# lucidrains/transfusion-pytorch

Measured on NVIDIA H100. Metric: train tokens/sec (text+latent) at d=512 L=8 seq=1024, higher is better.
Workload: dtype bf16

## Files before the change

### transfusion_pytorch_b200/csrc/gemm_sm90.cuh

```cuda
#pragma once
#include "sm90_ptx.cuh"
#include "dropout.cuh"

namespace tfx {

constexpr int GEMM_BM = 128;
constexpr int GEMM_BN = 128;
constexpr int GEMM_BK = 64;
constexpr int GEMM_UK = 16;

enum : int { EPI_STORE = 0, EPI_QKVG = 1, EPI_RESID = 2, EPI_GEGLU = 3, EPI_GEGLU_DROP = 4 };

struct GemmParams {
  int M, N, K;
  int k_splits;
  float* out_f32; long long ld_f32;
  __nv_bfloat16* out_bf16; long long ld_bf16;
  const float* bias;
  const long long* row_off;
  float alpha;
  int accumulate_f32;
  int K1;
  int H;
  __nv_bfloat16 *q, *k, *v;
  float* gates;
  float* mix_pre;
  float* qk_inv;
  const float *q_gamma, *k_gamma;
  const int* rope_pos;
  const float2* rope_cs;
  int rope_len;
  const int* kv_rows;
  const float* x_res; float* x_out; __nv_bfloat16* x_out_bf16;
  __nv_bfloat16* y_bf16;
  const int* cond_row;
  const float* zgate;
  long long zgate_ld;
  const float* ls;
  __nv_bfloat16* vg;
  __nv_bfloat16* h;
  DropParams drop;
};

template <int EPI> struct GemmCfg {
  static constexpr int THREADS = 384;
  static constexpr int STAGES = 4;
  static constexpr int A_BYTES = GEMM_BM * GEMM_BK * 2;
  static constexpr int B_BYTES = GEMM_BN * GEMM_BK * 2;
  static constexpr int STAGE_BYTES = A_BYTES + B_BYTES;
  static constexpr int ACC_BYTES = GEMM_BM * GEMM_BN * 4;
  static constexpr int STG_WARP = EPI == 2 ? 4096 + 2048 : 4096;
  static constexpr int STAGING = (EPI >= 3 ? 8 : 4) * STG_WARP;
  static constexpr int SMEM_BYTES = STAGES * STAGE_BYTES + ACC_BYTES + STAGING + 1024  + 256 ;
  static_assert(SMEM_BYTES <= 227 * 1024, "shared memory of one block");
};

__device__ __forceinline__ uint32_t acc_off(int r, int col) { return r * 512 + ((((col >> 2) ^ (r & 7))) << 4) + (col & 3) * 4; }
__device__ __forceinline__ void acc_ld32(const uint8_t* acc, int r, int col, uint32_t (&v)[32]) {
#pragma unroll
  for (int q = 0; q < 8; ++q) {
    const uint4 t = *reinterpret_cast<const uint4*>(acc + r * 512 + ((((col >> 2) + q) ^ (r & 7)) << 4));
    v[4 * q] = t.x; v[4 * q + 1] = t.y; v[4 * q + 2] = t.z; v[4 * q + 3] = t.w;
  }
}

__device__ __forceinline__ void gelu_parts(float g, float& cdf, float& pdf) {
  const float ax = fabsf(g) * 0.70710678118654752f;
  const float t = __fdividef(1.f, fmaf(0.3275911f, ax, 1.f));
  const float E = __expf(-ax * ax);
  float poly = fmaf(1.061405429f, t, -1.453152027f);
  poly = fmaf(poly, t, 1.421413741f);
  poly = fmaf(poly, t, -0.284496736f);
  poly = fmaf(poly, t, 0.254829592f);
  const float h = 0.5f * poly * t * E;
  cdf = g >= 0.f ? 1.f - h : h;
  pdf = 0.3989422804014327f * E;
}
__device__ __forceinline__ float gelu_erf(float x) { float c, d; gelu_parts(x, c, d); return x * c; }
__device__ __forceinline__ float2 geglu_pair(float2 g, float2 v) {
  return make_float2(gelu_erf(g.x) * v.x, gelu_erf(g.y) * v.y);
}

__device__ __forceinline__ void cp_async16_zfill(void* smem, const void* gmem, bool valid) {
  const int sz = valid ? 16 : 0;
  asm volatile("cp.async.cg.shared.global [%0], [%1], 16, %2;" ::"r"(smem_u32(smem)), "l"(gmem), "r"(sz) : "memory");
}

__device__ __forceinline__ uint32_t pack_bf16(float a, float b) {
  __nv_bfloat162 t = __floats2bfloat162_rn(a, b);
  return *reinterpret_cast<uint32_t*>(&t);
}
__device__ __forceinline__ float2 unpack2_bf16_(uint32_t w) {
  __nv_bfloat162 t = *reinterpret_cast<__nv_bfloat162*>(&w);
  return __bfloat1622float2(t);
}

template <int CH>
__device__ __forceinline__ void stg_put(uint8_t* sw, int lane, const uint32_t* w) {
#pragma unroll
  for (int c = 0; c < CH; ++c)
    *reinterpret_cast<uint4*>(sw + lane * 128 + ((c ^ (lane & 7)) << 4)) = make_uint4(w[4 * c], w[4 * c + 1], w[4 * c + 2], w[4 * c + 3]);
}
template <int CH>
__device__ __forceinline__ void stg_get(const uint8_t* sw, int lane, uint32_t* w) {
#pragma unroll
  for (int c = 0; c < CH; ++c) {
    const uint4 t = *reinterpret_cast<const uint4*>(sw + lane * 128 + ((c ^ (lane & 7)) << 4));
    w[4 * c] = t.x; w[4 * c + 1] = t.y; w[4 * c + 2] = t.z; w[4 * c + 3] = t.w;
  }
}
template <int CH>
__device__ __forceinline__ void stg_store(const uint8_t* sw, int lane, uint8_t* g, long long pitch, int rows_valid) {
  constexpr int RPI = 32 / CH;
#pragma unroll
  for (int it = 0; it < 32 / RPI; ++it) {
    const int row = it * RPI + lane / CH, ch = lane % CH;
    if (row < rows_valid)
      *reinterpret_cast<uint4*>(g + row * pitch + ch * 16) = *reinterpret_cast<const uint4*>(sw + row * 128 + ((ch ^ (row & 7)) << 4));
  }
}
__device__ __forceinline__ void stg_fetch(int lane, const uint8_t* g, long long pitch, int rows_valid, uint4 (&t)[8]) {
#pragma unroll
  for (int it = 0; it < 8; ++it) {
    const int row = it * 4 + lane / 8, ch = lane % 8;
    t[it] = row < rows_valid ? *reinterpret_cast<const uint4*>(g + row * pitch + ch * 16) : make_uint4(0, 0, 0, 0);
  }
}
__device__ __forceinline__ void stg_fill(uint8_t* sw, int lane, const uint4 (&t)[8]) {
#pragma unroll
  for (int it = 0; it < 8; ++it) {
    const int row = it * 4 + lane / 8, ch = lane % 8;
    *reinterpret_cast<uint4*>(sw + row * 128 + ((ch ^ (row & 7)) << 4)) = t[it];
  }
}

__device__ __forceinline__ void stg_put_pack(uint8_t* sw, int lane, const float* y) {
#pragma unroll
  for (int c = 0; c < 4; ++c)
    *reinterpret_cast<uint4*>(sw + lane * 128 + ((c ^ (lane & 7)) << 4)) =
        make_uint4(pack_bf16(y[8 * c], y[8 * c + 1]), pack_bf16(y[8 * c + 2], y[8 * c + 3]), pack_bf16(y[8 * c + 4], y[8 * c + 5]), pack_bf16(y[8 * c + 6], y[8 * c + 7]));
}
__device__ __forceinline__ void stg64_put(uint8_t* sw, int lane, const uint32_t* w) {
#pragma unroll
  for (int c = 0; c < 4; ++c)
    *reinterpret_cast<uint4*>(sw + lane * 64 + ((c ^ ((lane >> 1) & 3)) << 4)) = make_uint4(w[4 * c], w[4 * c + 1], w[4 * c + 2], w[4 * c + 3]);
}
__device__ __forceinline__ void stg64_put_pack(uint8_t* sw, int lane, const float* y) {
#pragma unroll
  for (int c = 0; c < 4; ++c)
    *reinterpret_cast<uint4*>(sw + lane * 64 + ((c ^ ((lane >> 1) & 3)) << 4)) =
        make_uint4(pack_bf16(y[8 * c], y[8 * c + 1]), pack_bf16(y[8 * c + 2], y[8 * c + 3]), pack_bf16(y[8 * c + 4], y[8 * c + 5]), pack_bf16(y[8 * c + 6], y[8 * c + 7]));
}
__device__ __forceinline__ void stg64_store(const uint8_t* sw, int lane, uint8_t* g, long long pitch, int rows_valid) {
#pragma unroll
  for (int it = 0; it < 4; ++it) {
    const int row = it * 8 + (lane >> 2), ch = lane & 3;
    if (row < rows_valid)
      *reinterpret_cast<uint4*>(g + row * pitch + ch * 16) = *reinterpret_cast<const uint4*>(sw + row * 64 + ((ch ^ ((row >> 1) & 3)) << 4));
  }
}

__device__ __forceinline__ void stg64_store_rows(const uint8_t* sw, int lane, uint8_t* g, long long pitch, int rows_valid, const int* __restrict__ rows) {
#pragma unroll
  for (int it = 0; it < 4; ++it) {
    const int row = it * 8 + (lane >> 2), ch = lane & 3;
    if (row < rows_valid)
      *reinterpret_cast<uint4*>(g + (long long)rows[row] * pitch + ch * 16) = *reinterpret_cast<const uint4*>(sw + row * 64 + ((ch ^ ((row >> 1) & 3)) << 4));
  }
}
template <int CH>
__device__ __forceinline__ void stg_store_rows(const uint8_t* sw, int lane, uint8_t* g, long long pitch, int rows_valid, const int* __restrict__ rows) {
  constexpr int RPI = 32 / CH;
#pragma unroll
  for (int it = 0; it < 32 / RPI; ++it) {
    const int row = it * RPI + lane / CH, ch = lane % CH;
    if (row < rows_valid)
      *reinterpret_cast<uint4*>(g + (long long)rows[row] * pitch + ch * 16) = *reinterpret_cast<const uint4*>(sw + row * 128 + ((ch ^ (row & 7)) << 4));
  }
}

template <class RowOf>
__device__ __forceinline__ void store_slice(const GemmParams& p, uint8_t* sw, int lane, uint32_t (&r)[32], int cbase, RowOf row_of) {
  const bool f32_staged = p.out_f32 && (p.row_off || (p.ld_f32 & 3) == 0) && ((reinterpret_cast<uintptr_t>(p.out_f32) & 15) == 0);
  const bool bf16_staged = p.out_bf16 && (p.ld_bf16 & 7) == 0 && ((reinterpret_cast<uintptr_t>(p.out_bf16) & 15) == 0);
  const int row = row_of(lane);
  const bool row_ok = row < p.M;
  const bool full = cbase + 32 <= p.N;
  float v[32];
#pragma unroll
  for (int j = 0; j < 32; ++j) v[j] = __uint_as_float(r[j]);
  if (p.alpha != 1.f) {
#pragma unroll
    for (int j = 0; j < 32; ++j) v[j] *= p.alpha;
  }
  if (p.bias) {
    if (full) {
#pragma unroll
      for (int j = 0; j < 32; j += 4) { const float4 b = *reinterpret_cast<const float4*>(p.bias + cbase + j); v[j] += b.x; v[j + 1] += b.y; v[j + 2] += b.z; v[j + 3] += b.w; }
    } else {
      for (int j = 0; j < 32; ++j) if (cbase + j < p.N) v[j] += p.bias[cbase + j];
    }
  }
  if (p.out_f32) {
    if (full && f32_staged) {
#pragma unroll
      for (int j = 0; j < 32; ++j) r[j] = __float_as_uint(v[j]);
      stg_put<8>(sw, lane, r);
      __syncwarp();
      auto put = [&](float* dst, float x) { if (p.accumulate_f32) atomicAdd(dst, x); else *dst = x; };
#pragma unroll
      for (int it = 0; it < 8; ++it) {
        const int rr = it * 4 + (lane >> 3), ch = lane & 7;
        const int grow = row_of(rr);
        if (grow < p.M) {
          const long long off = p.row_off ? p.row_off[grow] : (long long)grow * p.ld_f32;
          if (off >= 0) {
            float* drow = p.out_f32 + off + cbase;
            const uint8_t* srow = sw + rr * 128;
            const int a = (int)(reinterpret_cast<uintptr_t>(drow) >> 2) & 3;
            if (a == 0) {
              float* dst = drow + ch * 4;
              const float4 t = *reinterpret_cast<const float4*>(srow + ((ch ^ (rr & 7)) << 4));
              if (p.accumulate_f32) asm volatile("red.global.add.v4.f32 [%0], {%1, %2, %3, %4};" ::"l"(dst), "f"(t.x), "f"(t.y), "f"(t.z), "f"(t.w) : "memory");
              else *reinterpret_cast<float4*>(dst) = t;
            } else {
              const int pe = 4 - a;
              auto col = [&](int j) { return *reinterpret_cast<const float*>(srow + (((j >> 2) ^ (rr & 7)) << 4) + (j & 3) * 4); };
              if (ch < 7) {
                const int j = pe + 4 * ch;
                float* dst = drow + j;
                const float4 t = make_float4(col(j), col(j + 1), col(j + 2), col(j + 3));
                if (p.accumulate_f32) asm volatile("red.global.add.v4.f32 [%0], {%1, %2, %3, %4};" ::"l"(dst), "f"(t.x), "f"(t.y), "f"(t.z), "f"(t.w) : "memory");
                else *reinterpret_cast<float4*>(dst) = t;
              } else {
#pragma unroll
                for (int i = 0; i < 4; ++i) { const int j = i < pe ? i : 28 + i; put(drow + j, col(j)); }
              }
            }
          }
        }
      }
      __syncwarp();
    } else if (row_ok) {
      const long long off = p.row_off ? p.row_off[row] : (long long)row * p.ld_f32;
      if (off >= 0) {
        float* dst = p.out_f32 + off + cbase;
        for (int j = 0; j < 32; ++j)
          if (cbase + j < p.N) { if (p.accumulate_f32) atomicAdd(dst + j, v[j]); else dst[j] = v[j]; }
      }
    }
  }
  if (p.out_bf16) {
    if (full && bf16_staged) {
      uint32_t w[16];
#pragma unroll
      for (int j = 0; j < 16; ++j) w[j] = pack_bf16(v[2 * j], v[2 * j + 1]);
      stg_put<4>(sw, lane, w);
      __syncwarp();
#pragma unroll
      for (int it = 0; it < 4; ++it) {
        const int rr = it * 8 + (lane >> 2), ch = lane & 3;
        const int grow = row_of(rr);
        if (grow < p.M)
          *reinterpret_cast<uint4*>(p.out_bf16 + (long long)grow * p.ld_bf16 + cbase + ch * 8) = *reinterpret_cast<const uint4*>(sw + rr * 128 + ((ch ^ (rr & 7)) << 4));
      }
      __syncwarp();
    } else if (row_ok) {
      __nv_bfloat16* dst = p.out_bf16 + (long long)row * p.ld_bf16 + cbase;
      for (int j = 0; j < 32; ++j) if (cbase + j < p.N) dst[j] = __float2bfloat16(v[j]);
    }
  }
}

template <bool A_MN, bool B_MN, int EPI, int CL>
__global__ void __launch_bounds__(384, 1)
gemm_sm90_kernel(const __grid_constant__ CUtensorMap tmA, const __grid_constant__ CUtensorMap tmA2, const __grid_constant__ CUtensorMap tmB, const GemmParams p) {
  using Cfg = GemmCfg<EPI>;
  constexpr bool GEGLU = EPI == EPI_GEGLU || EPI == EPI_GEGLU_DROP;
  constexpr int BN = GEMM_BN;
  constexpr int STAGES = Cfg::STAGES;
  static_assert(Cfg::STAGE_BYTES % 1024 == 0 && 2 * STAGES <= 32, "stage alignment / barrier area");
  extern __shared__ __align__(1024) uint8_t smem_raw[];
  uint8_t* smem = smem_raw;
  if (threadIdx.x == 0 && (smem_u32(smem) & 1023u) != 0) __trap();
  uint8_t* acc = smem + STAGES * Cfg::STAGE_BYTES;
  uint8_t* staging = acc + Cfg::ACC_BYTES;
  uint64_t* bars = reinterpret_cast<uint64_t*>(staging + Cfg::STAGING);
  uint64_t* full_bar = bars;
  uint64_t* empty_bar = bars + STAGES;

  const int warp = threadIdx.x >> 5, lane = threadIdx.x & 31;
  const int m_tiles = (p.M + GEMM_BM - 1) / GEMM_BM;
  const int n_tiles = (p.N + BN - 1) / BN;
  const int kb_total = (p.K + GEMM_BK - 1) / GEMM_BK;
  const int kb_per_split = (kb_total + p.k_splits - 1) / p.k_splits;
  const int m_units = (m_tiles + CL - 1) / CL;
  const int unit_items = m_units * n_tiles;
  const int num_items = unit_items * p.k_splits;
  const int cta_rank = CL > 1 ? (int)cluster_ctarank() : 0;
  const int first_item = blockIdx.x / CL, item_stride = gridDim.x / CL;

  if (threadIdx.x == 0) {
    tma_prefetch_desc(&tmA);
    tma_prefetch_desc(&tmB);
    for (int s = 0; s < STAGES; ++s) { mbar_init(&full_bar[s], 1); mbar_init(&empty_bar[s], 4 * CL); }
    mbar_fence_init();
  }
  __syncthreads();
  if constexpr (CL > 1) cluster_sync_all();

  if (warp < 4) {
    setmaxnreg_dec<40>();
    if (threadIdx.x == 0) {
      int stage = 0; uint32_t phase = 0;
      for (int item = first_item; item < num_items; item += item_stride) {
        const int split = item / unit_items;
        const int rem = item - split * unit_items;
        const int m_unit = rem / n_tiles, n_blk = rem - m_unit * n_tiles;
        const int m_blk = m_unit * CL + cta_rank;
        const int kb0 = split * kb_per_split;
        const int kb1 = min(kb0 + kb_per_split, kb_total);
        for (int kb = kb0; kb < kb1; ++kb) {
          mbar_wait(&empty_bar[stage], phase ^ 1);
          uint8_t* sA = smem + stage * Cfg::STAGE_BYTES;
          uint8_t* sB = sA + Cfg::A_BYTES;
          mbar_expect_tx(&full_bar[stage], Cfg::STAGE_BYTES);
          if (!A_MN) {
            if (kb * GEMM_BK < p.K1) tma_load_2d(&tmA, &full_bar[stage], sA, kb * GEMM_BK, m_blk * GEMM_BM);
            else tma_load_2d(&tmA2, &full_bar[stage], sA, kb * GEMM_BK - p.K1, m_blk * GEMM_BM);
          } else {
#pragma unroll
            for (int a = 0; a < GEMM_BM / 64; ++a)
              tma_load_2d(&tmA, &full_bar[stage], sA + a * (GEMM_BK * 128), m_blk * GEMM_BM + a * 64, kb * GEMM_BK);
          }
          if constexpr (CL > 1) {
            if (!B_MN) tma_load_2d_multicast(&tmB, &full_bar[stage], sB + cta_rank * (64 * 128), kb * GEMM_BK, n_blk * BN + cta_rank * 64, (uint16_t)3);
            else tma_load_2d_multicast(&tmB, &full_bar[stage], sB + cta_rank * (GEMM_BK * 128), n_blk * BN + cta_rank * 64, kb * GEMM_BK, (uint16_t)3);
          } else if (!B_MN) {
            tma_load_2d(&tmB, &full_bar[stage], sB, kb * GEMM_BK, n_blk * BN);
          } else {
#pragma unroll
            for (int a = 0; a < BN / 64; ++a)
              tma_load_2d(&tmB, &full_bar[stage], sB + a * (GEMM_BK * 128), n_blk * BN + a * 64, kb * GEMM_BK);
          }
          if (++stage == STAGES) { stage = 0; phase ^= 1; }
        }
      }
    }
  } else {
    setmaxnreg_inc<232>();
    constexpr int BAR_TILE = 1, BAR_MMA = 3, BAR_ACC = 5;
    const int cw = (warp >> 2) - 1;
    const int quad = warp & 3;
    uint8_t* sw = staging + ((GEGLU ? 4 * cw : 0) + quad) * Cfg::STG_WARP;
    const int erow = quad * 32 + lane;
    int stage = 0; uint32_t phase = 0;
    auto release = [&](int s) {
      __syncwarp();
      if (lane == 0) {
        if constexpr (CL > 1) { mbar_arrive_cluster(&empty_bar[s], 0); mbar_arrive_cluster(&empty_bar[s], 1); }
        else mbar_arrive(&empty_bar[s]);
      }
    };
    int nth = 0;
    for (int item = first_item; item < num_items; item += item_stride, ++nth) {
      const int split = item / unit_items;
      const int rem = item - split * unit_items;
      const int m_unit = rem / n_tiles, n_blk = rem - m_unit * n_tiles;
      const int m_blk = m_unit * CL + cta_rank;
      const int kb0 = split * kb_per_split;
      const int kb1 = min(kb0 + kb_per_split, kb_total);
      if ((nth & 1) != cw) {
        const int s = stage + (kb1 - kb0);
        stage = s % STAGES;
        phase ^= (uint32_t)(s / STAGES) & 1u;
        continue;
      }
      const bool has_next = item + item_stride < num_items;
      if (nth > 0) named_bar_sync(BAR_MMA + cw, 256);
      float d0[64], d1[64];
#pragma unroll
      for (int i = 0; i < 64; ++i) { d0[i] = 0.f; d1[i] = 0.f; }
      int prev_stage = -1;
      for (int kb = kb0; kb < kb1; ++kb) {
        mbar_wait(&full_bar[stage], phase);
        const uint32_t sA = smem_u32(smem + stage * Cfg::STAGE_BYTES);
        const uint32_t sB = sA + Cfg::A_BYTES;
        wgmma_reg_fence(d0);
        wgmma_reg_fence(d1);
        wgmma_fence();
#pragma unroll
        for (int k = 0; k < GEMM_BK / GEMM_UK; ++k) {
          const uint64_t db = B_MN ? wgmma_desc_sw128(sB + k * (GEMM_UK * 128), GEMM_BK * 128, 1024)
                                   : wgmma_desc_sw128(sB + k * (GEMM_UK * 2), 16, 1024);
          const uint64_t da0 = A_MN ? wgmma_desc_sw128(sA + k * (GEMM_UK * 128), GEMM_BK * 128, 1024)
                                    : wgmma_desc_sw128(sA + k * (GEMM_UK * 2), 16, 1024);
          const uint64_t da1 = A_MN ? wgmma_desc_sw128(sA + GEMM_BK * 128 + k * (GEMM_UK * 128), GEMM_BK * 128, 1024)
                                    : wgmma_desc_sw128(sA + 64 * 128 + k * (GEMM_UK * 2), 16, 1024);
          const uint32_t acc_flag = (kb > kb0 || k > 0) ? 1u : 0u;
          wgmma_m64n128_ss<A_MN ? 1 : 0, B_MN ? 1 : 0>(d0, da0, db, acc_flag);
          wgmma_m64n128_ss<A_MN ? 1 : 0, B_MN ? 1 : 0>(d1, da1, db, acc_flag);
        }
        wgmma_commit();
        wgmma_wait<1>();
        if (prev_stage >= 0) release(prev_stage);
        prev_stage = stage;
        if (++stage == STAGES) { stage = 0; phase ^= 1; }
      }
      if (has_next) named_bar_arrive(BAR_MMA + (cw ^ 1), 256);
      wgmma_wait<0>();
      wgmma_reg_fence(d0);
      wgmma_reg_fence(d1);
      if (prev_stage >= 0) release(prev_stage);

      if (nth > 0) named_bar_sync(BAR_ACC + cw, 256);
      {
        const int r0 = quad * 16 + (lane >> 2);
#pragma unroll
        for (int q = 0; q < 16; ++q) {
          const int c = 8 * q + 2 * (lane & 3);
          *reinterpret_cast<float2*>(acc + acc_off(r0, c)) = make_float2(d0[4 * q], d0[4 * q + 1]);
          *reinterpret_cast<float2*>(acc + acc_off(r0 + 8, c)) = make_float2(d0[4 * q + 2], d0[4 * q + 3]);
          *reinterpret_cast<float2*>(acc + acc_off(r0 + 64, c)) = make_float2(d1[4 * q], d1[4 * q + 1]);
          *reinterpret_cast<float2*>(acc + acc_off(r0 + 72, c)) = make_float2(d1[4 * q + 2], d1[4 * q + 3]);
        }
      }
      named_bar_sync(BAR_TILE + cw, 128);

      const int wrow0 = m_blk * GEMM_BM + quad * 32;
      const int row = wrow0 + lane;
      const bool row_ok = row < p.M;
      const int rows_valid = min(32, p.M - wrow0);
      const int col0 = n_blk * BN;
      int qk_pos = 0;
      if constexpr (EPI == EPI_QKVG) { qk_pos = row_ok ? p.rope_pos[row] : 0; }
      if constexpr (EPI == EPI_RESID) { qk_pos = (row_ok && p.cond_row) ? p.cond_row[row] : -1; }

      if constexpr (EPI == EPI_STORE) {
#pragma unroll 1
        for (int c = 0; c < BN / 32; ++c) {
          const int cbase = col0 + c * 32;
          if (cbase >= p.N) break;
          uint32_t r[32];
          acc_ld32(acc, erow, c * 32, r);
          store_slice(p, sw, lane, r, cbase, [&](int i) { return wrow0 + i; });
        }
      } else if constexpr (EPI == EPI_QKVG) {
        const int tps = p.H >> 1;
        const int kind = n_blk / tps;
        const int tis = n_blk - kind * tps;
        const long long HI = (long long)p.H * 64;
        if (kind <= 1) {
          const float* gamma = kind == 0 ? p.q_gamma : p.k_gamma;
          __nv_bfloat16* dstm = kind == 0 ? p.q : p.k;
          const float2* cs = p.rope_cs + qk_pos;
#pragma unroll
          for (int hh = 0; hh < 2; ++hh) {
            uint32_t r0[32], r1[32];
            acc_ld32(acc, erow, hh * 64, r0);
            acc_ld32(acc, erow, hh * 64 + 32, r1);
            float ss = 0.f;
#pragma unroll
            for (int j = 0; j < 32; ++j) { float a = __uint_as_float(r0[j]), b = __uint_as_float(r1[j]); ss += a * a + b * b; }
            const float inv = 1.f / fmaxf(sqrtf(ss), 1e-12f);
            const int head = tis * 2 + hh;
            if (row_ok) p.qk_inv[(long long)row * 2 * p.H + kind * p.H + head] = inv;
            const float sc = inv * 8.f;
            uint32_t outw[32];
#pragma unroll
            for (int dh = 0; dh < 2; ++dh) {
              uint32_t* rr = dh == 0 ? r0 : r1;
#pragma unroll
              for (int i = 0; i < 16; ++i) {
                const int d0 = dh * 32 + 2 * i;
                const float2 gm = *reinterpret_cast<const float2*>(gamma + d0);
                const float y0 = __uint_as_float(rr[2 * i]) * sc * (gm.x + 1.f);
                const float y1 = __uint_as_float(rr[2 * i + 1]) * sc * (gm.y + 1.f);
                const float2 cc = cs[(long long)(dh * 16 + i) * p.rope_len];
                outw[dh * 16 + i] = pack_bf16(y0 * cc.x - y1 * cc.y, y1 * cc.x + y0 * cc.y);
              }
            }
            stg_put<8>(sw, lane, outw);
            __syncwarp();
            if (kind == 1 && p.kv_rows) stg_store_rows<8>(sw, lane, reinterpret_cast<uint8_t*>(dstm + head * 64), HI * 2, rows_valid, p.kv_rows + wrow0);
            else stg_store<8>(sw, lane, reinterpret_cast<uint8_t*>(dstm + (long long)wrow0 * HI + head * 64), HI * 2, rows_valid);
            __syncwarp();
          }
        } else if (kind == 2) {
#pragma unroll
          for (int c = 0; c < 2; ++c) {
            uint32_t r0[32], r1[32], w[32];
            acc_ld32(acc, erow, c * 64, r0);
            acc_ld32(acc, erow, c * 64 + 32, r1);
#pragma unroll
            for (int j = 0; j < 16; ++j) {
              w[j] = pack_bf16(__uint_as_float(r0[2 * j]), __uint_as_float(r0[2 * j + 1]));
              w[16 + j] = pack_bf16(__uint_as_float(r1[2 * j]), __uint_as_float(r1[2 * j + 1]));
            }
            stg_put<8>(sw, lane, w);
            __syncwarp();
            if (p.kv_rows) stg_store_rows<8>(sw, lane, reinterpret_cast<uint8_t*>(p.v + tis * 128 + c * 64), HI * 2, rows_valid, p.kv_rows + wrow0);
            else stg_store<8>(sw, lane, reinterpret_cast<uint8_t*>(p.v + (long long)wrow0 * HI + tis * 128 + c * 64), HI * 2, rows_valid);
            __syncwarp();
          }
        } else {
          uint32_t r[32];
          acc_ld32(acc, erow, 0, r);
          if (row_ok) {
            float* dst = p.gates + (long long)row * p.H;
#pragma unroll
            for (int j = 0; j < 32; ++j) if (j < p.H) dst[j] = __uint_as_float(r[j]);
            if (p.mix_pre) {
              float* dm = p.mix_pre + (long long)row * p.H;
#pragma unroll
              for (int j = 0; j < 32; ++j) if (j >= p.H && j < 2 * p.H) dm[j - p.H] = __uint_as_float(r[j]);
            }
          }
        }
      } else if constexpr (EPI == EPI_RESID) {
        const int crow = qk_pos;
        const float* zrow = (p.zgate && crow >= 0) ? p.zgate + (long long)crow * p.zgate_ld : nullptr;
        uint8_t* swb = sw + 4096;
        uint4 xres[8];
        auto fetch = [&](int sl) {
          stg_fetch(lane, reinterpret_cast<const uint8_t*>(p.x_res + (long long)wrow0 * p.N + col0 + sl * 32), (long long)p.N * 4,
                    col0 + sl * 32 < p.N ? rows_valid : 0, xres);
        };
        fetch(0);
#pragma unroll 1
        for (int sl = 0; sl < BN / 32; ++sl) {
          const int cbase = col0 + sl * 32;
          if (cbase >= p.N) break;
          __syncwarp();
          stg_fill(sw, lane, xres);
          if (sl + 1 < BN / 32) fetch(sl + 1);
          uint32_t r[32];
          acc_ld32(acc, erow, sl * 32, r);
          float y[32];
#pragma unroll
          for (int j = 0; j < 32; ++j) y[j] = __uint_as_float(r[j]);
          if (p.bias) {
#pragma unroll
            for (int j = 0; j < 32; j += 4) { const float4 b = *reinterpret_cast<const float4*>(p.bias + cbase + j); y[j] += b.x; y[j + 1] += b.y; y[j + 2] += b.z; y[j + 3] += b.w; }
          }
          if (p.y_bf16) {
            stg64_put_pack(swb, lane, y);
            __syncwarp();
            stg64_store(swb, lane, reinterpret_cast<uint8_t*>(p.y_bf16 + (long long)wrow0 * p.N + cbase), (long long)p.N * 2, rows_valid);
            __syncwarp();
          }
          {
            uint32_t xrv[32];
            __syncwarp();
            stg_get<8>(sw, lane, xrv);
            if (zrow) {
#pragma unroll
              for (int j = 0; j < 32; j += 4) {
                const float4 s4 = *reinterpret_cast<const float4*>(zrow + cbase + j);
                y[j] = __uint_as_float(xrv[j]) + y[j] * s4.x; y[j + 1] = __uint_as_float(xrv[j + 1]) + y[j + 1] * s4.y;
                y[j + 2] = __uint_as_float(xrv[j + 2]) + y[j + 2] * s4.z; y[j + 3] = __uint_as_float(xrv[j + 3]) + y[j + 3] * s4.w;
              }
            } else if (p.ls) {
#pragma unroll
              for (int j = 0; j < 32; j += 4) {
                const float4 s4 = *reinterpret_cast<const float4*>(p.ls + cbase + j);
                y[j] = __uint_as_float(xrv[j]) + y[j] * (s4.x + 1.f); y[j + 1] = __uint_as_float(xrv[j + 1]) + y[j + 1] * (s4.y + 1.f);
                y[j + 2] = __uint_as_float(xrv[j + 2]) + y[j + 2] * (s4.z + 1.f); y[j + 3] = __uint_as_float(xrv[j + 3]) + y[j + 3] * (s4.w + 1.f);
              }
            } else {
#pragma unroll
              for (int j = 0; j < 32; ++j) y[j] += __uint_as_float(xrv[j]);
            }
          }
          if (p.x_out)
#pragma unroll
          for (int hfc = 0; hfc < 2; ++hfc) {
            uint32_t w16[16];
#pragma unroll
            for (int j = 0; j < 16; ++j) w16[j] = __float_as_uint(y[hfc * 16 + j]);
            __syncwarp();
            stg64_put(swb, lane, w16);
            __syncwarp();
            stg64_store(swb, lane, reinterpret_cast<uint8_t*>(p.x_out + (long long)wrow0 * p.N + cbase + hfc * 16), (long long)p.N * 4, rows_valid);
          }
          if (p.x_out_bf16) {
            __syncwarp();
            stg64_put_pack(swb, lane, y);
            __syncwarp();
            stg64_store(swb, lane, reinterpret_cast<uint8_t*>(p.x_out_bf16 + (long long)wrow0 * p.N + cbase), (long long)p.N * 2, rows_valid);
          }
          __syncwarp();
        }
      } else if constexpr (GEGLU) {
        uint32_t keep[2] = {0u, 0u};
        if constexpr (EPI == EPI_GEGLU_DROP) {
          const uint32_t k0 = __ldg(p.drop.key), k1 = __ldg(p.drop.key + 1);
#pragma unroll
          for (int q = 0; q < 8; ++q) keep[q >> 2] |= drop_keep8(p.drop, k0, k1, DROP_SITE_FFN, 0, (uint32_t)row, (uint32_t)(n_blk * 8 + q)) << (8 * (q & 3));
        }
        uint32_t ra[4][32];
#pragma unroll
        for (int q = 0; q < 4; ++q) acc_ld32(acc, erow, q * 32, ra[q]);
        if (has_next) named_bar_arrive(BAR_ACC + (cw ^ 1), 256);
#pragma unroll
        for (int c = 0; c < 2; ++c) {
          const int cv = col0 + c * 32, cg = cv + 64;
          if (cv >= p.N) break;
          float v[32], g[32];
#pragma unroll
          for (int j = 0; j < 32; ++j) { v[j] = __uint_as_float(ra[c][j]) + p.bias[cv + j]; g[j] = __uint_as_float(ra[2 + c][j]) + p.bias[cg + j]; }
          __syncwarp();
          stg64_put_pack(sw, lane, v);
          __syncwarp();
          stg64_store(sw, lane, reinterpret_cast<uint8_t*>(p.vg + (long long)wrow0 * p.N + cv), (long long)p.N * 2, rows_valid);
          __syncwarp();
          stg64_put_pack(sw, lane, g);
          __syncwarp();
          stg64_store(sw, lane, reinterpret_cast<uint8_t*>(p.vg + (long long)wrow0 * p.N + cg), (long long)p.N * 2, rows_valid);
#pragma unroll
          for (int j = 0; j < 32; j += 2) {
            const float2 o = geglu_pair(make_float2(g[j], g[j + 1]), make_float2(v[j], v[j + 1]));
            g[j] = o.x; g[j + 1] = o.y;
          }
          if constexpr (EPI == EPI_GEGLU_DROP) {
#pragma unroll
            for (int j = 0; j < 32; ++j) g[j] = (keep[c] >> j) & 1u ? g[j] * p.drop.scale : 0.f;
          }
          __syncwarp();
          stg64_put_pack(sw, lane, g);
          __syncwarp();
          stg64_store(sw, lane, reinterpret_cast<uint8_t*>(p.h + (long long)wrow0 * (p.N / 2) + n_blk * 64 + c * 32), (long long)p.N, rows_valid);
          __syncwarp();
        }
      }
      if (!GEGLU && has_next) named_bar_arrive(BAR_ACC + (cw ^ 1), 256);
    }
  }
  if constexpr (CL > 1) {
    __syncthreads();
    cluster_sync_all();
  }
}

struct GemmWideCfg {
  static constexpr int BM = 256;
  static constexpr int THREADS = 384;
  static constexpr int STAGES = 4;
  static constexpr int A_BYTES = BM * GEMM_BK * 2;
  static constexpr int B_BYTES = GEMM_BN * GEMM_BK * 2;
  static constexpr int STAGE_BYTES = A_BYTES + B_BYTES;
  static constexpr int STAGING = 8 * 4096;
  static constexpr int SMEM_BYTES = STAGES * STAGE_BYTES + STAGING + 1024  + 256 ;
  static_assert(SMEM_BYTES <= 227 * 1024, "shared memory of one block");
};

template <bool A_MN, bool B_MN>
__global__ void __launch_bounds__(384, 1)
gemm_sm90_wide_kernel(const __grid_constant__ CUtensorMap tmA, const __grid_constant__ CUtensorMap tmB, const GemmParams p) {
  using Cfg = GemmWideCfg;
  constexpr int BM = Cfg::BM, BN = GEMM_BN, STAGES = Cfg::STAGES;
  static_assert(Cfg::STAGE_BYTES % 1024 == 0, "stage alignment");
  extern __shared__ __align__(1024) uint8_t smem_raw[];
  uint8_t* smem = smem_raw;
  if (threadIdx.x == 0 && (smem_u32(smem) & 1023u) != 0) __trap();
  uint8_t* staging = smem + STAGES * Cfg::STAGE_BYTES;
  uint64_t* full_bar = reinterpret_cast<uint64_t*>(staging + Cfg::STAGING);
  uint64_t* empty_bar = full_bar + STAGES;

  const int warp = threadIdx.x >> 5, lane = threadIdx.x & 31;
  const int m_tiles = (p.M + BM - 1) / BM;
  const int n_tiles = (p.N + BN - 1) / BN;
  const int kb_total = (p.K + GEMM_BK - 1) / GEMM_BK;
  const int kb_per_split = (kb_total + p.k_splits - 1) / p.k_splits;
  const int tiles = m_tiles * n_tiles;
  const int num_items = tiles * p.k_splits;

  if (threadIdx.x == 0) {
    tma_prefetch_desc(&tmA);
    tma_prefetch_desc(&tmB);
    for (int s = 0; s < STAGES; ++s) { mbar_init(&full_bar[s], 1); mbar_init(&empty_bar[s], 8); }
    mbar_fence_init();
  }
  __syncthreads();

  if (warp < 4) {
    setmaxnreg_dec<40>();
    if (threadIdx.x == 0) {
      int stage = 0; uint32_t phase = 0;
      for (int item = blockIdx.x; item < num_items; item += gridDim.x) {
        const int split = item / tiles;
        const int rem = item - split * tiles;
        const int m_blk = rem / n_tiles, n_blk = rem - m_blk * n_tiles;
        const int kb0 = split * kb_per_split;
        const int kb1 = min(kb0 + kb_per_split, kb_total);
        for (int kb = kb0; kb < kb1; ++kb) {
          mbar_wait(&empty_bar[stage], phase ^ 1);
          uint8_t* sA = smem + stage * Cfg::STAGE_BYTES;
          uint8_t* sB = sA + Cfg::A_BYTES;
          mbar_expect_tx(&full_bar[stage], Cfg::STAGE_BYTES);
          if (!A_MN) {
            tma_load_2d(&tmA, &full_bar[stage], sA, kb * GEMM_BK, m_blk * BM);
          } else {
#pragma unroll
            for (int a = 0; a < BM / 64; ++a)
              tma_load_2d(&tmA, &full_bar[stage], sA + a * (GEMM_BK * 128), m_blk * BM + a * 64, kb * GEMM_BK);
          }
          if (!B_MN) {
            tma_load_2d(&tmB, &full_bar[stage], sB, kb * GEMM_BK, n_blk * BN);
          } else {
#pragma unroll
            for (int a = 0; a < BN / 64; ++a)
              tma_load_2d(&tmB, &full_bar[stage], sB + a * (GEMM_BK * 128), n_blk * BN + a * 64, kb * GEMM_BK);
          }
          if (++stage == STAGES) { stage = 0; phase ^= 1; }
        }
      }
    }
  } else {
    setmaxnreg_inc<232>();
    const int cw = (warp >> 2) - 1;
    const int quad = warp & 3;
    uint8_t* sw = staging + (4 * cw + quad) * 4096;
    const uint32_t a_half = (uint32_t)cw * (A_MN ? 2 * GEMM_BK * 128 : 128 * 128);
    int stage = 0; uint32_t phase = 0;
    auto release = [&](int s) { __syncwarp(); if (lane == 0) mbar_arrive(&empty_bar[s]); };
    for (int item = blockIdx.x; item < num_items; item += gridDim.x) {
      const int split = item / tiles;
      const int rem = item - split * tiles;
      const int m_blk = rem / n_tiles, n_blk = rem - m_blk * n_tiles;
      const int kb0 = split * kb_per_split;
      const int kb1 = min(kb0 + kb_per_split, kb_total);
      float d0[64], d1[64];
#pragma unroll
      for (int i = 0; i < 64; ++i) { d0[i] = 0.f; d1[i] = 0.f; }
      int prev_stage = -1;
      for (int kb = kb0; kb < kb1; ++kb) {
        mbar_wait(&full_bar[stage], phase);
        const uint32_t sA = smem_u32(smem + stage * Cfg::STAGE_BYTES) + a_half;
        const uint32_t sB = smem_u32(smem + stage * Cfg::STAGE_BYTES) + Cfg::A_BYTES;
        wgmma_reg_fence(d0);
        wgmma_reg_fence(d1);
        wgmma_fence();
#pragma unroll
        for (int k = 0; k < GEMM_BK / GEMM_UK; ++k) {
          const uint64_t db = B_MN ? wgmma_desc_sw128(sB + k * (GEMM_UK * 128), GEMM_BK * 128, 1024)
                                   : wgmma_desc_sw128(sB + k * (GEMM_UK * 2), 16, 1024);
          const uint64_t da0 = A_MN ? wgmma_desc_sw128(sA + k * (GEMM_UK * 128), GEMM_BK * 128, 1024)
                                    : wgmma_desc_sw128(sA + k * (GEMM_UK * 2), 16, 1024);
          const uint64_t da1 = A_MN ? wgmma_desc_sw128(sA + GEMM_BK * 128 + k * (GEMM_UK * 128), GEMM_BK * 128, 1024)
                                    : wgmma_desc_sw128(sA + 64 * 128 + k * (GEMM_UK * 2), 16, 1024);
          const uint32_t acc_flag = (kb > kb0 || k > 0) ? 1u : 0u;
          wgmma_m64n128_ss<A_MN ? 1 : 0, B_MN ? 1 : 0>(d0, da0, db, acc_flag);
          wgmma_m64n128_ss<A_MN ? 1 : 0, B_MN ? 1 : 0>(d1, da1, db, acc_flag);
        }
        wgmma_commit();
        wgmma_wait<1>();
        if (prev_stage >= 0) release(prev_stage);
        prev_stage = stage;
        if (++stage == STAGES) { stage = 0; phase ^= 1; }
      }
      wgmma_wait<0>();
      wgmma_reg_fence(d0);
      wgmma_reg_fence(d1);
      if (prev_stage >= 0) release(prev_stage);

      const int wrow0 = m_blk * BM + 128 * cw + 16 * quad;
      const int r0 = lane >> 2;
#pragma unroll
      for (int c = 0; c < BN / 32; ++c) {
        const int cbase = n_blk * BN + c * 32;
        if (cbase >= p.N) break;
#pragma unroll
        for (int q4 = 0; q4 < 4; ++q4) {
          const int q = 4 * c + q4, col = 8 * q4 + 2 * (lane & 3);
          auto put2 = [&](int rr, float x, float y) {
            *reinterpret_cast<float2*>(sw + rr * 128 + ((((col >> 2) ^ (rr & 7))) << 4) + (col & 3) * 4) = make_float2(x, y);
          };
          put2(r0, d0[4 * q], d0[4 * q + 1]);
          put2(r0 + 8, d0[4 * q + 2], d0[4 * q + 3]);
          put2(r0 + 16, d1[4 * q], d1[4 * q + 1]);
          put2(r0 + 24, d1[4 * q + 2], d1[4 * q + 3]);
        }
        __syncwarp();
        uint32_t r[32];
        stg_get<8>(sw, lane, r);
        __syncwarp();
        store_slice(p, sw, lane, r, cbase, [&](int i) { return wrow0 + (i & 15) + ((i >> 4) << 6); });
      }
    }
  }
}

typedef CUresult (*PFN_encodeTiled)(CUtensorMap*, CUtensorMapDataType, cuuint32_t, void*, const cuuint64_t*, const cuuint64_t*,
                                    const cuuint32_t*, const cuuint32_t*, CUtensorMapInterleave, CUtensorMapSwizzle,
                                    CUtensorMapL2promotion, CUtensorMapFloatOOBfill);

inline PFN_encodeTiled get_encode_fn() {
  static PFN_encodeTiled fn = nullptr;
  if (!fn) {
    void* f = nullptr;
    cudaDriverEntryPointQueryResult qres;
    if (cudaGetDriverEntryPoint("cuTensorMapEncodeTiled", &f, cudaEnableDefault, &qres) != cudaSuccess || !f) return nullptr;
    fn = reinterpret_cast<PFN_encodeTiled>(f);
  }
  return fn;
}

inline int make_tmap_bf16(CUtensorMap* tm, const void* ptr, long long inner, long long outer, long long ld, int box_rows) {
  PFN_encodeTiled enc = get_encode_fn();
  if (!enc) return -1;
  cuuint64_t dims[2] = {(cuuint64_t)inner, (cuuint64_t)outer};
  cuuint64_t strides[1] = {(cuuint64_t)ld * 2};
  cuuint32_t box[2] = {64, (cuuint32_t)box_rows};
  cuuint32_t estr[2] = {1, 1};
  CUresult r = enc(tm, CU_TENSOR_MAP_DATA_TYPE_BFLOAT16, 2, const_cast<void*>(ptr), dims, strides, box, estr,
                   CU_TENSOR_MAP_INTERLEAVE_NONE, CU_TENSOR_MAP_SWIZZLE_128B, CU_TENSOR_MAP_L2_PROMOTION_L2_256B,
                   CU_TENSOR_MAP_FLOAT_OOB_FILL_NONE);
  return r == CUDA_SUCCESS ? 0 : -(int)r - 1000;
}

struct GemmOperand {
  const void* ptr;
  long long ld;
  bool mn_major;
  const void* ptr2 = nullptr;
  long long ld2 = 0;
};

inline int& gemm_cluster_mode_ref() {
  static int mode = -1;
  if (mode < 0) { const char* e = getenv("TFX_GEMM_CLUSTER"); mode = e ? atoi(e) : 1; }
  return mode;
}

inline int gemm_effective_splits(int K, int k_splits) {
  const int kbt = (K + GEMM_BK - 1) / GEMM_BK;
  int s = k_splits < 1 ? 1 : k_splits > kbt ? kbt : k_splits;
  const int per = (kbt + s - 1) / s;
  return (kbt + per - 1) / per;
}
inline int gemm_kb_per_item(int K, int k_splits) { return ((K + GEMM_BK - 1) / GEMM_BK + k_splits - 1) / k_splits; }

constexpr int GEMM_WIDE_MIN_KB = 16;
inline int& gemm_wide_mode_ref() { static int mode = 1; return mode; }
inline bool gemm_store_wide(int K, int k_splits) {
  const int mode = gemm_wide_mode_ref();
  if (mode != 1) return mode == 2;
  return gemm_cluster_mode_ref() == 1 && gemm_kb_per_item(K, gemm_effective_splits(K, k_splits)) >= GEMM_WIDE_MIN_KB;
}

template <bool A_MN, bool B_MN>
int launch_gemm_wide_t(const GemmOperand& A, const GemmOperand& B, const GemmParams& p_in, int num_sms, cudaStream_t stream) {
  using Cfg = GemmWideCfg;
  GemmParams p = p_in;
  p.K1 = p.K;
  p.k_splits = gemm_effective_splits(p.K, p.k_splits);
  const int items = ((p.M + Cfg::BM - 1) / Cfg::BM) * ((p.N + GEMM_BN - 1) / GEMM_BN) * p.k_splits;
  if (items <= 0) return 0;
  CUtensorMap tmA, tmB;
  int rc = !A_MN ? make_tmap_bf16(&tmA, A.ptr, p.K, p.M, A.ld, Cfg::BM) : make_tmap_bf16(&tmA, A.ptr, p.M, p.K, A.ld, GEMM_BK);
  if (rc) return rc;
  rc = !B_MN ? make_tmap_bf16(&tmB, B.ptr, p.K, p.N, B.ld, GEMM_BN) : make_tmap_bf16(&tmB, B.ptr, p.N, p.K, B.ld, GEMM_BK);
  if (rc) return rc;
  auto kern = gemm_sm90_wide_kernel<A_MN, B_MN>;
  static bool attr_set = false;
  if (!attr_set) {
    if (cudaFuncSetAttribute(kern, cudaFuncAttributeMaxDynamicSharedMemorySize, Cfg::SMEM_BYTES) != cudaSuccess) return -2;
    attr_set = true;
  }
  const int grid = items < num_sms ? items : num_sms;
  kern<<<grid, Cfg::THREADS, Cfg::SMEM_BYTES, stream>>>(tmA, tmB, p);
  return cudaGetLastError() == cudaSuccess ? 0 : -3;
}

template <bool A_MN, bool B_MN, int EPI>
int launch_gemm_t(const GemmOperand& A, const GemmOperand& B, const GemmParams& p_in, int num_sms, cudaStream_t stream) {
  using Cfg = GemmCfg<EPI>;
  GemmParams p = p_in;
  CUtensorMap tmA, tmA2, tmB;
  int rc;
  const bool two = (!A_MN) && A.ptr2 != nullptr;
  if (!two) p.K1 = p.K;
  if (!A_MN) rc = make_tmap_bf16(&tmA, A.ptr, two ? p.K1 : p.K, p.M, A.ld, GEMM_BM); else rc = make_tmap_bf16(&tmA, A.ptr, p.M, p.K, A.ld, GEMM_BK);
  if (rc) return rc;
  if (two) { rc = make_tmap_bf16(&tmA2, A.ptr2, p.K - p.K1, p.M, A.ld2, GEMM_BM); if (rc) return rc; } else tmA2 = tmA;
  p.k_splits = gemm_effective_splits(p.K, p.k_splits);
  const int m_tiles = (p.M + GEMM_BM - 1) / GEMM_BM, n_tiles = (p.N + GEMM_BN - 1) / GEMM_BN;
  const int items = m_tiles * n_tiles * p.k_splits;
  if (items <= 0) return 0;
  const int mode = gemm_cluster_mode_ref();
  const int kb_item = gemm_kb_per_item(p.K, p.k_splits);
  const bool paired = mode == 2 || (mode == 3 && m_tiles >= 2 && kb_item >= 16 && items >= 2 * num_sms);
  if (!B_MN) rc = make_tmap_bf16(&tmB, B.ptr, p.K, p.N, B.ld, paired ? GEMM_BN / 2 : GEMM_BN); else rc = make_tmap_bf16(&tmB, B.ptr, p.N, p.K, B.ld, GEMM_BK);
  if (rc) return rc;
  if (paired) {
    auto kern = gemm_sm90_kernel<A_MN, B_MN, EPI, 2>;
    static int max_clusters = 0;
    cudaLaunchConfig_t cfg;
    memset(&cfg, 0, sizeof(cfg));
    cudaLaunchAttribute at[1];
    at[0].id = cudaLaunchAttributeClusterDimension;
    at[0].val.clusterDim.x = 2; at[0].val.clusterDim.y = 1; at[0].val.clusterDim.z = 1;
    cfg.blockDim = dim3(Cfg::THREADS); cfg.dynamicSmemBytes = Cfg::SMEM_BYTES; cfg.stream = stream; cfg.attrs = at; cfg.numAttrs = 1;
    if (!max_clusters) {
      if (cudaFuncSetAttribute(kern, cudaFuncAttributeMaxDynamicSharedMemorySize, Cfg::SMEM_BYTES) != cudaSuccess) return -2;
      cfg.gridDim = dim3(2 * (num_sms / 2));
      int nc = 0;
      if (cudaOccupancyMaxActiveClusters(&nc, kern, &cfg) != cudaSuccess || nc < 1) { cudaGetLastError(); nc = num_sms / 2; }
      max_clusters = nc < num_sms / 2 ? nc : num_sms / 2;
    }
    const int pair_items = ((m_tiles + 1) / 2) * n_tiles * p.k_splits;
    const int clusters = pair_items < max_clusters ? pair_items : max_clusters;
    cfg.gridDim = dim3(2 * clusters);
    return cudaLaunchKernelEx(&cfg, kern, tmA, tmA2, tmB, p) == cudaSuccess ? 0 : -3;
  }
  auto kern = gemm_sm90_kernel<A_MN, B_MN, EPI, 1>;
  static bool attr_set = false;
  if (!attr_set) {
    if (cudaFuncSetAttribute(kern, cudaFuncAttributeMaxDynamicSharedMemorySize, Cfg::SMEM_BYTES) != cudaSuccess) return -2;
    attr_set = true;
  }
  const int grid = items < num_sms ? items : num_sms;
  kern<<<grid, Cfg::THREADS, Cfg::SMEM_BYTES, stream>>>(tmA, tmA2, tmB, p);
  return cudaGetLastError() == cudaSuccess ? 0 : -3;
}

}
```

Baseline: 1.228 million.

## Move residual GEMM epilogue to per-warp fragment staging with async residual prefetch

For the residual-add epilogue, accumulator fragments are no longer spilled into a shared 128x128 fp32 tile behind named barriers. Each warp now transposes its own register fragments through a private staging slab and processes rows in a slab layout. The residual input is prefetched with cp.async into shared memory, overlapping the next slice's load with the current slice's arithmetic. This removes the accumulator buffer and cross-warpgroup barrier synchronisation for that epilogue, at the cost of more staging memory per warp and a more intricate row mapping. The wide GEMM path reuses the new fragment helper.

```diff
diff --git a/transfusion_pytorch_b200/csrc/gemm_sm90.cuh b/transfusion_pytorch_b200/csrc/gemm_sm90.cuh
--- a/transfusion_pytorch_b200/csrc/gemm_sm90.cuh
+++ b/transfusion_pytorch_b200/csrc/gemm_sm90.cuh
@@ -48,9 +48,9 @@
   static constexpr int A_BYTES = GEMM_BM * GEMM_BK * 2;
   static constexpr int B_BYTES = GEMM_BN * GEMM_BK * 2;
   static constexpr int STAGE_BYTES = A_BYTES + B_BYTES;
-  static constexpr int ACC_BYTES = GEMM_BM * GEMM_BN * 4;
-  static constexpr int STG_WARP = EPI == 2 ? 4096 + 2048 : 4096;
-  static constexpr int STAGING = (EPI >= 3 ? 8 : 4) * STG_WARP;
+  static constexpr int ACC_BYTES = EPI == 2 ? 0 : GEMM_BM * GEMM_BN * 4;
+  static constexpr int STG_WARP = EPI == 2 ? 2 * 4096 : 4096;
+  static constexpr int STAGING = (EPI >= 2 ? 8 : 4) * STG_WARP;
   static constexpr int SMEM_BYTES = STAGES * STAGE_BYTES + ACC_BYTES + STAGING + 1024  + 256 ;
   static_assert(SMEM_BYTES <= 227 * 1024, "shared memory of one block");
 };
@@ -95,6 +95,10 @@
   return __bfloat1622float2(t);
 }
 
+__device__ __forceinline__ int slab_row(int i) { return (i & 15) + ((i >> 4) << 6); }
+
+__device__ __forceinline__ int lane_now() { int l; asm volatile("mov.u32 %0, %%laneid;" : "=r"(l)); return l; }
+
 template <int CH>
 __device__ __forceinline__ void stg_put(uint8_t* sw, int lane, const uint32_t* w) {
 #pragma unroll
@@ -119,21 +123,6 @@
       *reinterpret_cast<uint4*>(g + row * pitch + ch * 16) = *reinterpret_cast<const uint4*>(sw + row * 128 + ((ch ^ (row & 7)) << 4));
   }
 }
-__device__ __forceinline__ void stg_fetch(int lane, const uint8_t* g, long long pitch, int rows_valid, uint4 (&t)[8]) {
-#pragma unroll
-  for (int it = 0; it < 8; ++it) {
-    const int row = it * 4 + lane / 8, ch = lane % 8;
-    t[it] = row < rows_valid ? *reinterpret_cast<const uint4*>(g + row * pitch + ch * 16) : make_uint4(0, 0, 0, 0);
-  }
-}
-__device__ __forceinline__ void stg_fill(uint8_t* sw, int lane, const uint4 (&t)[8]) {
-#pragma unroll
-  for (int it = 0; it < 8; ++it) {
-    const int row = it * 4 + lane / 8, ch = lane % 8;
-    *reinterpret_cast<uint4*>(sw + row * 128 + ((ch ^ (row & 7)) << 4)) = t[it];
-  }
-}
-
 __device__ __forceinline__ void stg_put_pack(uint8_t* sw, int lane, const float* y) {
 #pragma unroll
   for (int c = 0; c < 4; ++c)
@@ -157,6 +146,39 @@
     const int row = it * 8 + (lane >> 2), ch = lane & 3;
     if (row < rows_valid)
       *reinterpret_cast<uint4*>(g + row * pitch + ch * 16) = *reinterpret_cast<const uint4*>(sw + row * 64 + ((ch ^ ((row >> 1) & 3)) << 4));
+  }
+}
+
+__device__ __forceinline__ void frag_slice(uint8_t* sw, const float (&d0)[64], const float (&d1)[64], int c, uint32_t (&r)[32]) {
+  const int lane = lane_now();
+  const int r0 = lane >> 2;
+  const int off = r0 * 128 + ((((lane >> 1) & 1) ^ r0) << 4) + (lane & 1) * 8;
+#pragma unroll
+  for (int q4 = 0; q4 < 4; ++q4) {
+    const int q = 4 * c + q4;
+    uint8_t* a = sw + (off ^ (q4 << 5));
+    *reinterpret_cast<float2*>(a) = make_float2(d0[4 * q], d0[4 * q + 1]);
+    *reinterpret_cast<float2*>(a + 1024) = make_float2(d0[4 * q + 2], d0[4 * q + 3]);
+    *reinterpret_cast<float2*>(a + 2048) = make_float2(d1[4 * q], d1[4 * q + 1]);
+    *reinterpret_cast<float2*>(a + 3072) = make_float2(d1[4 * q + 2], d1[4 * q + 3]);
+  }
+  __syncwarp();
+  const int roff = lane * 128 + ((lane & 7) << 4);
+#pragma unroll
+  for (int j = 0; j < 8; ++j) {
+    const uint4 t = *reinterpret_cast<const uint4*>(sw + (roff ^ (j << 4)));
+    r[4 * j] = t.x; r[4 * j + 1] = t.y; r[4 * j + 2] = t.z; r[4 * j + 3] = t.w;
+  }
+  __syncwarp();
+}
+
+__device__ __forceinline__ void stg64_store_slab(const uint8_t* sw, int lane, uint8_t* g, int pitch, int rows_valid) {
+  lane = lane_now();
+#pragma unroll
+  for (int it = 0; it < 4; ++it) {
+    const int row = it * 8 + (lane >> 2), ch = lane & 3;
+    if (slab_row(row) < rows_valid)
+      *reinterpret_cast<uint4*>(g + slab_row(row) * pitch + ch * 16) = *reinterpret_cast<const uint4*>(sw + row * 64 + ((ch ^ ((row >> 1) & 3)) << 4));
   }
 }
 
@@ -352,7 +374,7 @@
     constexpr int BAR_TILE = 1, BAR_MMA = 3, BAR_ACC = 5;
     const int cw = (warp >> 2) - 1;
     const int quad = warp & 3;
-    uint8_t* sw = staging + ((GEGLU ? 4 * cw : 0) + quad) * Cfg::STG_WARP;
+    uint8_t* sw = staging + ((EPI >= EPI_RESID ? 4 * cw : 0) + quad) * Cfg::STG_WARP;
     const int erow = quad * 32 + lane;
     int stage = 0; uint32_t phase = 0;
     auto release = [&](int s) {
@@ -413,8 +435,8 @@
       wgmma_reg_fence(d1);
       if (prev_stage >= 0) release(prev_stage);
 
-      if (nth > 0) named_bar_sync(BAR_ACC + cw, 256);
-      {
+      if constexpr (EPI != EPI_RESID) {
+        if (nth > 0) named_bar_sync(BAR_ACC + cw, 256);
         const int r0 = quad * 16 + (lane >> 2);
 #pragma unroll
         for (int q = 0; q < 16; ++q) {
@@ -424,13 +446,14 @@
           *reinterpret_cast<float2*>(acc + acc_off(r0 + 64, c)) = make_float2(d1[4 * q], d1[4 * q + 1]);
           *reinterpret_cast<float2*>(acc + acc_off(r0 + 72, c)) = make_float2(d1[4 * q + 2], d1[4 * q + 3]);
         }
-      }
-      named_bar_sync(BAR_TILE + cw, 128);
-
-      const int wrow0 = m_blk * GEMM_BM + quad * 32;
-      const int row = wrow0 + lane;
+        named_bar_sync(BAR_TILE + cw, 128);
+      }
+
+      constexpr bool FRAG = EPI == EPI_RESID;
+      const int wrow0 = m_blk * GEMM_BM + (FRAG ? quad * 16 : quad * 32);
+      const int row = wrow0 + (FRAG ? slab_row(lane) : lane);
       const bool row_ok = row < p.M;
-      const int rows_valid = min(32, p.M - wrow0);
+      const int rows_valid = FRAG ? p.M - wrow0 : min(32, p.M - wrow0);
       const int col0 = n_blk * BN;
       int qk_pos = 0;
       if constexpr (EPI == EPI_QKVG) { qk_pos = row_ok ? p.rope_pos[row] : 0; }
@@ -520,22 +543,27 @@
       } else if constexpr (EPI == EPI_RESID) {
         const int crow = qk_pos;
         const float* zrow = (p.zgate && crow >= 0) ? p.zgate + (long long)crow * p.zgate_ld : nullptr;
-        uint8_t* swb = sw + 4096;
-        uint4 xres[8];
+        uint8_t* swx = sw + 4096;
         auto fetch = [&](int sl) {
-          stg_fetch(lane, reinterpret_cast<const uint8_t*>(p.x_res + (long long)wrow0 * p.N + col0 + sl * 32), (long long)p.N * 4,
-                    col0 + sl * 32 < p.N ? rows_valid : 0, xres);
+          const int lane = lane_now();
+          const uint8_t* g = reinterpret_cast<const uint8_t*>(p.x_res + (long long)wrow0 * p.N + col0 + sl * 32);
+          const int l8 = lane / 8, ch = lane % 8;
+          const int off = l8 * 128 + ((ch ^ l8) << 4);
+#pragma unroll
+          for (int it = 0; it < 8; ++it) {
+            const int rr = it * 4 + l8;
+            const bool ok = slab_row(rr) < rows_valid;
+            cp_async16_zfill(swx + (off ^ ((it & 1) << 6)) + 512 * it, ok ? g + (long long)slab_row(rr) * p.N * 4 + ch * 16 : g, ok);
+          }
+          asm volatile("cp.async.commit_group;" ::: "memory");
         };
         fetch(0);
-#pragma unroll 1
+#pragma unroll
         for (int sl = 0; sl < BN / 32; ++sl) {
           const int cbase = col0 + sl * 32;
           if (cbase >= p.N) break;
-          __syncwarp();
-          stg_fill(sw, lane, xres);
-          if (sl + 1 < BN / 32) fetch(sl + 1);
           uint32_t r[32];
-          acc_ld32(acc, erow, sl * 32, r);
+          frag_slice(sw, d0, d1, sl, r);
           float y[32];
 #pragma unroll
           for (int j = 0; j < 32; ++j) y[j] = __uint_as_float(r[j]);
@@ -544,50 +572,61 @@
             for (int j = 0; j < 32; j += 4) { const float4 b = *reinterpret_cast<const float4*>(p.bias + cbase + j); y[j] += b.x; y[j + 1] += b.y; y[j + 2] += b.z; y[j + 3] += b.w; }
           }
           if (p.y_bf16) {
-            stg64_put_pack(swb, lane, y);
+            stg64_put_pack(sw, lane, y);
             __syncwarp();
-            stg64_store(swb, lane, reinterpret_cast<uint8_t*>(p.y_bf16 + (long long)wrow0 * p.N + cbase), (long long)p.N * 2, rows_valid);
+            stg64_store_slab(sw, lane, reinterpret_cast<uint8_t*>(p.y_bf16 + (long long)wrow0 * p.N + cbase), (long long)p.N * 2, rows_valid);
             __syncwarp();
           }
-          {
-            uint32_t xrv[32];
-            __syncwarp();
-            stg_get<8>(sw, lane, xrv);
+          asm volatile("cp.async.wait_group 0;" ::: "memory");
+          __syncwarp();
+#pragma unroll
+          for (int hfc = 0; hfc < 2; ++hfc) {
+            const int cb = cbase + 16 * hfc;
+            float* yh = y + 16 * hfc;
+            uint32_t xrv[16];
+            {
+              const int ln = lane_now(), off = ln * 128 + ((ln & 7) << 4);
+#pragma unroll
+              for (int c = 0; c < 4; ++c) {
+                const uint4 t = *reinterpret_cast<const uint4*>(swx + (off ^ ((4 * hfc + c) << 4)));
+                xrv[4 * c] = t.x; xrv[4 * c + 1] = t.y; xrv[4 * c + 2] = t.z; xrv[4 * c + 3] = t.w;
+              }
+            }
             if (zrow) {
 #pragma unroll
-              for (int j = 0; j < 32; j += 4) {
-                const float4 s4 = *reinterpret_cast<const float4*>(zrow + cbase + j);
-                y[j] = __uint_as_float(xrv[j]) + y[j] * s4.x; y[j + 1] = __uint_as_float(xrv[j + 1]) + y[j + 1] * s4.y;
-                y[j + 2] = __uint_as_float(xrv[j + 2]) + y[j + 2] * s4.z; y[j + 3] = __uint_as_float(xrv[j + 3]) + y[j + 3] * s4.w;
+              for (int j = 0; j < 16; j += 4) {
+                const float4 s4 = *reinterpret_cast<const float4*>(zrow + cb + j);
+                yh[j] = __uint_as_float(xrv[j]) + yh[j] * s4.x; yh[j + 1] = __uint_as_float(xrv[j + 1]) + yh[j + 1] * s4.y;
+                yh[j + 2] = __uint_as_float(xrv[j + 2]) + yh[j + 2] * s4.z; yh[j + 3] = __uint_as_float(xrv[j + 3]) + yh[j + 3] * s4.w;
               }
             } else if (p.ls) {
 #pragma unroll
-              for (int j = 0; j < 32; j += 4) {
-                const float4 s4 = *reinterpret_cast<const float4*>(p.ls + cbase + j);
-                y[j] = __uint_as_float(xrv[j]) + y[j] * (s4.x + 1.f); y[j + 1] = __uint_as_float(xrv[j + 1]) + y[j + 1] * (s4.y + 1.f);
-                y[j + 2] = __uint_as_float(xrv[j + 2]) + y[j + 2] * (s4.z + 1.f); y[j + 3] = __uint_as_float(xrv[j + 3]) + y[j + 3] * (s4.w + 1.f);
+              for (int j = 0; j < 16; j += 4) {
+                const float4 s4 = *reinterpret_cast<const float4*>(p.ls + cb + j);
+                yh[j] = __uint_as_float(xrv[j]) + yh[j] * (s4.x + 1.f); yh[j + 1] = __uint_as_float(xrv[j + 1]) + yh[j + 1] * (s4.y + 1.f);
+                yh[j + 2] = __uint_as_float(xrv[j + 2]) + yh[j + 2] * (s4.z + 1.f); yh[j + 3] = __uint_as_float(xrv[j + 3]) + yh[j + 3] * (s4.w + 1.f);
               }
             } else {
 #pragma unroll
-              for (int j = 0; j < 32; ++j) y[j] += __uint_as_float(xrv[j]);
+              for (int j = 0; j < 16; ++j) yh[j] += __uint_as_float(xrv[j]);
             }
-          }
-          if (p.x_out)
-#pragma unroll
-          for (int hfc = 0; hfc < 2; ++hfc) {
-            uint32_t w16[16];
-#pragma unroll
-            for (int j = 0; j < 16; ++j) w16[j] = __float_as_uint(y[hfc * 16 + j]);
+            if (p.x_out) {
+              uint32_t w16[16];
+#pragma unroll
+              for (int j = 0; j < 16; ++j) w16[j] = __float_as_uint(yh[j]);
+              __syncwarp();
+              stg64_put(sw, lane, w16);
+              __syncwarp();
+              stg64_store_slab(sw, lane, reinterpret_cast<uint8_t*>(p.x_out + (long long)wrow0 * p.N + cb), (long long)p.N * 4, rows_valid);
+            }
             __syncwarp();
-            stg64_put(swb, lane, w16);
-            __syncwarp();
-            stg64_store(swb, lane, reinterpret_cast<uint8_t*>(p.x_out + (long long)wrow0 * p.N + cbase + hfc * 16), (long long)p.N * 4, rows_valid);
-          }
+          }
+          if (sl + 1 < BN / 32 && cbase + 32 < p.N) fetch(sl + 1);
           if (p.x_out_bf16) {
             __syncwarp();
-            stg64_put_pack(swb, lane, y);
+            stg64_put_pack(sw, lane, y);
             __syncwarp();
-            stg64_store(swb, lane, reinterpret_cast<uint8_t*>(p.x_out_bf16 + (long long)wrow0 * p.N + cbase), (long long)p.N * 2, rows_valid);
+            stg64_store_slab(sw, lane, reinterpret_cast<uint8_t*>(p.x_out_bf16 + (long long)wrow0 * p.N + cbase), (long long)p.N * 2, rows_valid);
           }
           __syncwarp();
         }
@@ -633,7 +672,7 @@
           __syncwarp();
         }
       }
-      if (!GEGLU && has_next) named_bar_arrive(BAR_ACC + (cw ^ 1), 256);
+      if (!GEGLU && !FRAG && has_next) named_bar_arrive(BAR_ACC + (cw ^ 1), 256);
     }
   }
   if constexpr (CL > 1) {
@@ -765,27 +804,13 @@
       if (prev_stage >= 0) release(prev_stage);
 
       const int wrow0 = m_blk * BM + 128 * cw + 16 * quad;
-      const int r0 = lane >> 2;
 #pragma unroll
       for (int c = 0; c < BN / 32; ++c) {
         const int cbase = n_blk * BN + c * 32;
         if (cbase >= p.N) break;
-#pragma unroll
-        for (int q4 = 0; q4 < 4; ++q4) {
-          const int q = 4 * c + q4, col = 8 * q4 + 2 * (lane & 3);
-          auto put2 = [&](int rr, float x, float y) {
-            *reinterpret_cast<float2*>(sw + rr * 128 + ((((col >> 2) ^ (rr & 7))) << 4) + (col & 3) * 4) = make_float2(x, y);
-          };
-          put2(r0, d0[4 * q], d0[4 * q + 1]);
-          put2(r0 + 8, d0[4 * q + 2], d0[4 * q + 3]);
-          put2(r0 + 16, d1[4 * q], d1[4 * q + 1]);
-          put2(r0 + 24, d1[4 * q + 2], d1[4 * q + 3]);
-        }
-        __syncwarp();
         uint32_t r[32];
-        stg_get<8>(sw, lane, r);
-        __syncwarp();
-        store_slice(p, sw, lane, r, cbase, [&](int i) { return wrow0 + (i & 15) + ((i >> 4) << 6); });
+        frag_slice(sw, d0, d1, c, r);
+        store_slice(p, sw, lane, r, cbase, [&](int i) { return wrow0 + slab_row(i); });
       }
     }
   }
```

After: 1.233 million, median of 6. No clear change (+0.4%).
